# HasnainRaz/Fast-SRGAN

Hardware: AMD Instinct MI355X
Metric: SR train-step images/sec (96->384 4x, full GAN step: G+D+VGG perceptual loss) (higher is better)
Workload: dtype x3v; 1 GPU; BASELINE configs[2]: full GAN training step, 8 residual blocks / 64 filters, 96x96->384x384; per_gpu_batch=32, global_batch=32, parallelism=dp1, collectives=none, rccl_world_size=1, launch=hipGraph replay

## Files before the change

### fast-srgan_amd/csrc/conv_wgrad.hip

```cpp
#include "fsr_common.h"
#include "fsr_host.h"
#include <cstdlib>

constexpr int WGRAD_GROUP_MAX = 32;

#ifndef FSR_ABLW
#define FSR_ABLW 0
#endif

struct WgradKArgs {
  const void* x;
  const void* dy;
  float* ws;
  int N, IH, IW, CinPad;
  int OH, OW, CoutPad;
  int dy_ps;
  int tiles_x, tiles_y, tiles_total, tiles_per_slab, nslab;
  int nbm, nbn;
  int x3;
  int group_n;
  const void* gx[WGRAD_GROUP_MAX];
  const void* gdy[WGRAD_GROUP_MAX];
};

struct WgradGroupOut {
  float* dw[WGRAD_GROUP_MAX];
};

template <typename T, int BM, int BN, int S, int TPH>
constexpr bool wgrad_dma() {
  return sizeof(T) == 2 && BM >= 64 && BN == 64 && (S == 1 || TPH == 4);
}
template <typename T, int BM, int BN, int S, int TPH>
constexpr int wgrad_dma_dy_instr() {
  return (TPH * 16 * ((BM + 16) / (16 / (int)sizeof(T))) + 63) / 64;
}
template <typename T, int BM, int BN, int S, int TPH>
constexpr int wgrad_dma_halo_instr() {
  return (((TPH - 1) * S + 3) * (15 * S + 3) * ((BN + 16) / (16 / (int)sizeof(T))) + 63) / 64;
}
template <typename T, int BM, int BN, int S, int TPH>
constexpr size_t wgrad_dma_lds_bytes() {
  return (size_t)2 * 1024 * (wgrad_dma_dy_instr<T, BM, BN, S, TPH>() + wgrad_dma_halo_instr<T, BM, BN, S, TPH>());
}

template <typename T, int BM, int BN, int S, int TPH, bool X3W = false>
__global__ __launch_bounds__((BM >= 64 && BN == 64) ? 512 : 256) void conv_wgrad_kernel(const WgradKArgs a) {
  static_assert(!X3W || (BM == 128 && BN == 64 && sizeof(T) == 2), "the x3 form of the 128 x 64 block");
  constexpr int NW = (BM >= 64 && BN == 64) ? 8 : 4;
  static_assert(BM <= 64 || (BM == 128 && BN == 64 && sizeof(T) == 2), "128-row blocks: 16-bit, 64 input channels");
  constexpr int NTHR = NW * 64;
  constexpr int EPB = 16 / (int)sizeof(T);
  constexpr int PAD = 16;
  constexpr int PA = BM + PAD, PB = BN + PAD;
  constexpr int HH = (TPH - 1) * S + 3, HW = 15 * S + 3;
  constexpr int NPAIR = (BM / 16) * (BN / 16);
  constexpr int TPW = (NPAIR + NW - 1) / NW;
  constexpr int NBT = BN / 16;
  static_assert(TPW <= NBT, "a wave's pairs must share its co tile");
  constexpr int TPIX = TPH * 16;

  HIP_DYNAMIC_SHARED(char, smem)
  T* dyt = (T*)smem;
  T* halo = dyt + TPIX * PA;
  constexpr bool DMA = wgrad_dma<T, BM, BN, S, TPH>();

  const int tid = threadIdx.x, lane = tid & 63, wave = __builtin_amdgcn_readfirstlane(tid >> 6);
  const int l15 = lane & 15, lg = lane >> 4;
  int bid = a.group_n > 0 ? (int)blockIdx.x : xcd_remap((int)blockIdx.x, (int)gridDim.x);
  const int layer = a.group_n > 0 ? bid / a.nslab : 0;
  if (a.group_n > 0) bid -= layer * a.nslab;
  const int bn = bid % a.nbn;
  bid /= a.nbn;
  const int bm = bid % a.nbm;
  const int slab = bid / a.nbm;

  constexpr bool COPAIR = (BM >= 64 && BN == 64);
  const bool active = wave * TPW < NPAIR;
  const int co_t = COPAIR ? (wave / NBT) * TPW : (wave * TPW) / NBT;
  constexpr bool x3blk = X3W;
  const int ci_t0 = COPAIR ? (x3blk ? (wave + 2 * (wave / NBT)) % NBT : wave % NBT) : (wave * TPW) % NBT;
  const bool skip_lo = x3blk && ci_t0 >= 2;

  f32x4 acc[9][TPW];
#pragma unroll
  for (int t = 0; t < 9; ++t)
#pragma unroll
    for (int j = 0; j < TPW; ++j) acc[t][j] = (f32x4){0.f, 0.f, 0.f, 0.f};

  const void* xsel = a.x;
  const void* dysel = a.dy;
  if (a.group_n > 0) {
#pragma unroll
    for (int l = 0; l < WGRAD_GROUP_MAX; ++l)
      if (l == layer) {
        xsel = a.gx[l];
        dysel = a.gdy[l];
      }
  }
  const T* xg = (const T*)xsel;
  const T* dyg = (const T*)dysel;
  const int tile0 = slab * a.tiles_per_slab;
  const int tile1 = (tile0 + a.tiles_per_slab < a.tiles_total) ? tile0 + a.tiles_per_slab : a.tiles_total;

  constexpr int DUNITS = TPIX * (BM / EPB), HUNITS = HH * HW * (BN / EPB);
  constexpr int DPT = (DUNITS + NTHR - 1) / NTHR, HPT = (HUNITS + NTHR - 1) / NTHR;
  u32x4 dreg[DPT], hreg[HPT];
  auto stage_issue = [&](int tile) {
    const int tx = tile % a.tiles_x;
    const int ty = (tile / a.tiles_x) % a.tiles_y;
    const int img = tile / (a.tiles_x * a.tiles_y);
    const int oy0 = ty * TPH, ox0 = tx * 16;
#pragma unroll
    for (int i = 0; i < DPT; ++i) {
      const int u = tid + i * NTHR;
      u32x4 v = (u32x4){0u, 0u, 0u, 0u};
      if (DUNITS % NTHR == 0 || u < DUNITS) {
        const int unit = u % (BM / EPB), p = u / (BM / EPB);
        const int oy = oy0 + p / 16, ox = ox0 + (p & 15);
        if (oy < a.OH && ox < a.OW) {
          const int ch = bm * BM + unit * EPB;
          unsigned eoff;
          if (!a.dy_ps) {
            eoff = (unsigned)((img * a.OH + oy) * a.OW + ox) * (unsigned)a.CoutPad + (unsigned)ch;
          } else {
            const int cps = a.CoutPad >> 2;
            const int q = ch / cps, cc = ch - q * cps;
            eoff = (unsigned)((img * 2 * a.OH + 2 * oy + (q >> 1)) * (2 * a.OW) + 2 * ox + (q & 1)) * (unsigned)cps + (unsigned)cc;
          }
          v = *(const u32x4*)(dyg + eoff);
        }
      }
      dreg[i] = v;
    }
    const int iy0 = oy0 * S - 1, ix0 = ox0 * S - 1;
#pragma unroll
    for (int i = 0; i < HPT; ++i) {
      const int u = tid + i * NTHR;
      u32x4 v = (u32x4){0u, 0u, 0u, 0u};
      if (HUNITS % NTHR == 0 || u < HUNITS) {
        const int unit = u % (BN / EPB), p = u / (BN / EPB);
        const int iy = iy0 + p / HW, ix = ix0 + p % HW;
        if (iy >= 0 && iy < a.IH && ix >= 0 && ix < a.IW)
          v = *(const u32x4*)(xg + (unsigned)((img * a.IH + iy) * a.IW + ix) * (unsigned)a.CinPad + (unsigned)(bn * BN + unit * EPB));
      }
      hreg[i] = v;
    }
  };
  auto stage_commit = [&]() {
#pragma unroll
    for (int i = 0; i < DPT; ++i) {
      const int u = tid + i * NTHR;
      if (DUNITS % NTHR == 0 || u < DUNITS) *(u32x4*)(dyt + (u / (BM / EPB)) * PA + (u % (BM / EPB)) * EPB) = dreg[i];
    }
#pragma unroll
    for (int i = 0; i < HPT; ++i) {
      const int u = tid + i * NTHR;
      if (HUNITS % NTHR == 0 || u < HUNITS) *(u32x4*)(halo + (u / (BN / EPB)) * PB + (u % (BN / EPB)) * EPB) = hreg[i];
    }
  };

  constexpr int UPA = PA / EPB, UPB = PB / EPB;
  constexpr int DYI = wgrad_dma_dy_instr<T, BM, BN, S, TPH>(), HAI = wgrad_dma_halo_instr<T, BM, BN, S, TPH>();
  constexpr int NPIECE = DYI + HAI, IPW = (NPIECE + NW - 1) / NW;
  constexpr unsigned IMG_BYTES = NPIECE * 1024u;
  unsigned rel[DMA ? IPW : 1], pk[DMA ? IPW : 1];
  if constexpr (DMA) {
#pragma unroll
    for (int j = 0; j < IPW; ++j) {
      const int g = j * NW + wave;
      unsigned r_ = 0, k_ = 0x80000000u;
      if (g < DYI) {
        const int slot = g * 64 + lane, p_ = slot / UPA, u_ = slot - p_ * UPA;
        const int py = p_ >> 4, px = p_ & 15;
        const int ch = bm * BM + u_ * EPB;
        if (!a.dy_ps) {
          r_ = (unsigned)((py * a.OW + px) * a.CoutPad + ch);
        } else {
          const int cps = a.CoutPad >> 2;
          const int q = ch / cps, cc = ch - q * cps;
          r_ = (unsigned)(((2 * py + (q >> 1)) * (2 * a.OW) + 2 * px + (q & 1)) * cps + cc);
        }
        k_ = (unsigned)py | ((unsigned)px << 8) | ((u_ >= BM / EPB || p_ >= TPIX) ? 0x80000000u : 0u);
      } else if (g < NPIECE) {
        const int slot = (g - DYI) * 64 + lane, p_ = slot / UPB, u_ = slot - p_ * UPB;
        const int py = p_ / HW, px = p_ - py * HW;
        r_ = (unsigned)((py * a.IW + px) * a.CinPad + bn * BN + u_ * EPB);
        k_ = (unsigned)py | ((unsigned)px << 8) | ((u_ >= BN / EPB || p_ >= HH * HW) ? 0x80000000u : 0u);
      }
      rel[j] = r_;
      pk[j] = k_;
    }
  }
  const fsr_buf_t dy_buf = fsr_make_buf(dyg, DMA ? (unsigned)((size_t)a.N * a.OH * a.OW * a.CoutPad * sizeof(T)) : 0u);
  const fsr_buf_t x_buf = fsr_make_buf(xg, DMA ? (unsigned)((size_t)a.N * a.IH * a.IW * a.CinPad * sizeof(T)) : 0u);
  const fsr_lds_addr_t lds0 = FSR_LDS_ADDR(smem);
  struct DmaTile {
    int oy0, ox0, iy0, ix0;
    unsigned dy_base, x_base;
    fsr_lds_addr_t lds;
    bool on;
  };
  auto dma_tile = [&](int tile, int image, bool on) {
    DmaTile d;
    const int tx = tile % a.tiles_x;
    const int ty = (tile / a.tiles_x) % a.tiles_y;
    const int img = tile / (a.tiles_x * a.tiles_y);
    d.oy0 = ty * TPH;
    d.ox0 = tx * 16;
    d.dy_base = !a.dy_ps ? (unsigned)((img * a.OH + d.oy0) * a.OW + d.ox0) * (unsigned)a.CoutPad
                         : (unsigned)((img * 2 * a.OH + 2 * d.oy0) * (2 * a.OW) + 2 * d.ox0) * (unsigned)(a.CoutPad >> 2);
    d.iy0 = d.oy0 * S - 1;
    d.ix0 = d.ox0 * S - 1;
    d.x_base = (unsigned)((img * a.IH + d.iy0) * a.IW + d.ix0) * (unsigned)a.CinPad;
    d.lds = lds0 + (fsr_lds_addr_t)(image * IMG_BYTES);
    d.on = on;
    return d;
  };
  auto dma_piece = [&](const DmaTile& d, int j) {
    const int g = j * NW + wave;
    if (!d.on || (NPIECE % NW != 0 && g >= NPIECE)) return;
    const int py = (int)(pk[j] & 0xffu), px = (int)((pk[j] >> 8) & 0xffu);
#if FSR_ABLW == 7
    const bool keep = false;
// ... 10 lines not shown
      FSR_BLDS16(x_buf, voff, 0u, d.lds + (fsr_lds_addr_t)(g * 1024));
    }
  };
  auto dma_issue = [&](int tile, int image) {
    const DmaTile d = dma_tile(tile, image, true);
#pragma unroll
    for (int j = 0; j < IPW; ++j) dma_piece(d, j);
  };

  int image = 0;
  if constexpr (DMA) {
    if (tile0 < tile1) dma_issue(tile0, 0);
  } else {
    if (tile0 < tile1) stage_issue(tile0);
  }
  for (int tile = tile0; tile < tile1; ++tile) {
    if constexpr (DMA) {
#if FSR_ABLW != 4 && FSR_ABLW != 6
      FSR_WAIT_VM(0);
#endif
#if FSR_ABLW != 5 && FSR_ABLW != 6
      FSR_BARRIER();
#endif
#if FSR_ABLW != 1
      if (tile + 1 < tile1) dma_issue(tile + 1, image ^ 1);
#endif
      dyt = (T*)(smem + image * IMG_BYTES);
      halo = (T*)(smem + image * IMG_BYTES + DYI * 1024);
      image ^= 1;
    } else {
      __syncthreads();
#if FSR_ABLW == 1
      if (tile == tile0) stage_commit();
      __syncthreads();
#else
      stage_commit();
      __syncthreads();
      if (tile + 1 < tile1) stage_issue(tile + 1);
#endif
    }
    if (!active) continue;
#if FSR_ABLW == 2
    continue;
#endif

    if constexpr (sizeof(T) == 2 && COPAIR) {
      constexpr int NS = TPH / 2, NSTAGE = NS * 9;
      const int qrow = l15 >> 2, qch = (l15 & 3) * 4, c0 = 8 * (lg & 1);
      const T* pa_base = dyt + ((lg >> 1) * 16 + c0 + qrow) * PA + co_t * 16 + qch;
      const T* pb_base = halo + ((lg >> 1) * S * HW + (c0 + qrow) * S) * PB + ci_t0 * 16 + qch;
      auto frag = [&](const T* p0, int second) {
        const s16x4 lo = __builtin_amdgcn_ds_read_tr16_b64_v4i16(FSR_LDS_PTR(s16x4, p0));
        const s16x4 hi = __builtin_amdgcn_ds_read_tr16_b64_v4i16(FSR_LDS_PTR(s16x4, p0 + second));
        return (s16x8){lo[0], lo[1], lo[2], lo[3], hi[0], hi[1], hi[2], hi[3]};
      };
      auto xfrag = [&](int i) {
        const int ks = i / 9, t = i % 9;
        return frag(pb_base + ((ks * 2 * S + t / 3) * HW + t % 3) * PB, 4 * S * PB);
      };
      constexpr int NWH = (BM == 128) ? 2 : TPW;
      s16x8 af[2][TPW], bf[3];
#pragma unroll
      for (int w = 0; w < TPW; ++w) af[0][w] = frag(pa_base + w * 16, 4 * PA);
      bf[0] = xfrag(0);
      bf[1] = xfrag(1);
#pragma unroll
      for (int i = 0; i < NSTAGE; ++i) {
        const int ks = i / 9, t = i % 9;
        if (i + 2 < NSTAGE) bf[(i + 2) % 3] = xfrag(i + 2);
        if (t == 4 && ks + 1 < NS) {
#pragma unroll
          for (int w = 0; w < NWH; ++w) af[(ks + 1) & 1][w] = frag(pa_base + (ks + 1) * 32 * PA + w * 16, 4 * PA);
          if (!skip_lo) {
#pragma unroll
            for (int w = NWH; w < TPW; ++w) af[(ks + 1) & 1][w] = frag(pa_base + (ks + 1) * 32 * PA + w * 16, 4 * PA);
          }
        }
#pragma unroll
        for (int w = 0; w < NWH; ++w) acc[t][w] = mfma16<T>(af[ks & 1][w], bf[i % 3], acc[t][w]);
        if (!skip_lo) {
#pragma unroll
          for (int w = NWH; w < TPW; ++w) acc[t][w] = mfma16<T>(af[ks & 1][w], bf[i % 3], acc[t][w]);
        }
        __builtin_amdgcn_sched_barrier(0);
      }
    } else if constexpr (sizeof(T) == 2) {
      const int qrow = l15 >> 2, qch = (l15 & 3) * 4;
#pragma unroll 1
      for (int s = 0; s < TPH / 2; ++s) {
        const int r = 2 * s + (lg >> 1);
        const int c0 = 8 * (lg & 1);
        constexpr int NA = COPAIR ? TPW : 1;
        s16x8 af[NA];
#pragma unroll
        for (int w = 0; w < NA; ++w) {
          const T* pa = dyt + (r * 16 + c0 + qrow) * PA + (co_t + w) * 16 + qch;
          const s16x4 lo = __builtin_amdgcn_ds_read_tr16_b64_v4i16(FSR_LDS_PTR(s16x4, pa));
          const s16x4 hi = __builtin_amdgcn_ds_read_tr16_b64_v4i16(FSR_LDS_PTR(s16x4, pa + 4 * PA));
          af[w] = (s16x8){lo[0], lo[1], lo[2], lo[3], hi[0], hi[1], hi[2], hi[3]};
        }
#pragma unroll
        for (int t = 0; t < 9; ++t) {
          const int ky = t / 3, kx = t % 3;
          const T* pb0 = halo + ((r * S + ky) * HW + (c0 + qrow) * S + kx) * PB + ci_t0 * 16 + qch;
          if constexpr (COPAIR) {
#if FSR_ABLW == 3
            const s16x8 bf = af[(t + 1) & 1];
#else
            const s16x4 lo = __builtin_amdgcn_ds_read_tr16_b64_v4i16(FSR_LDS_PTR(s16x4, pb0));
            const s16x4 hi = __builtin_amdgcn_ds_read_tr16_b64_v4i16(FSR_LDS_PTR(s16x4, pb0 + 4 * S * PB));
            const s16x8 bf = (s16x8){lo[0], lo[1], lo[2], lo[3], hi[0], hi[1], hi[2], hi[3]};
#endif
#pragma unroll
            for (int w = 0; w < TPW; ++w) acc[t][w] = mfma16<T>(af[w], bf, acc[t][w]);
          } else {
#pragma unroll
            for (int j = 0; j < TPW; ++j) {
              const s16x4 lo = __builtin_amdgcn_ds_read_tr16_b64_v4i16(FSR_LDS_PTR(s16x4, pb0 + j * 16));
              const s16x4 hi = __builtin_amdgcn_ds_read_tr16_b64_v4i16(FSR_LDS_PTR(s16x4, pb0 + j * 16 + 4 * S * PB));
              const s16x8 bf = (s16x8){lo[0], lo[1], lo[2], lo[3], hi[0], hi[1], hi[2], hi[3]};
              acc[t][j] = mfma16<T>(af[0], bf, acc[t][j]);
            }
          }
        }
      }
    } else {
#pragma unroll 1
      for (int s = 0; s < TPH * 4; ++s) {
        const int r = s >> 2, c = 4 * (s & 3) + lg;
        const float av = dyt[(r * 16 + c) * PA + co_t * 16 + l15];
        const float av1 = COPAIR ? dyt[(r * 16 + c) * PA + (co_t + 1) * 16 + l15] : 0.f;
#pragma unroll
        for (int t = 0; t < 9; ++t) {
          const int ky = t / 3, kx = t % 3;
          const T* pb = halo + ((r * S + ky) * HW + c * S + kx) * PB + ci_t0 * 16 + l15;
          if constexpr (COPAIR) {
            const float bv = pb[0];
            acc[t][0] = mfma_f32_16x16x4(av, bv, acc[t][0]);
            acc[t][1] = mfma_f32_16x16x4(av1, bv, acc[t][1]);
          } else {
#pragma unroll
            for (int j = 0; j < TPW; ++j) acc[t][j] = mfma_f32_16x16x4(av, pb[j * 16], acc[t][j]);
          }
        }
      }
    }
  }

  if (!active) return;
#pragma unroll
  for (int t = 0; t < 9; ++t)
#pragma unroll
    for (int j = 0; j < TPW; ++j) {
      const int cot = COPAIR ? co_t + j : co_t, cit = COPAIR ? ci_t0 : ci_t0 + j;
      float* o = a.ws + (((size_t)(layer * a.nslab + slab) * 9 + t) * a.CoutPad + bm * BM + cot * 16 + lg * 4) * a.CinPad + bn * BN + cit * 16 + l15;
#pragma unroll
      for (int r = 0; r < 4; ++r) o[(size_t)r * a.CinPad] = acc[t][j][r];
    }
}

__global__ __launch_bounds__(256) void conv_wgrad_reduce_kernel(const float* __restrict__ ws, float* __restrict__ dw, int nslab,
                                                                int cout, int cin, int cout_pad, int cin_pad, int ps) {
  __shared__ float red[8][32];
  const int total = 9 * cout * cin;
  const size_t sstride = (size_t)9 * cout_pad * cin_pad;
  const int oi = threadIdx.x & 31, pl = threadIdx.x >> 5;
  for (int i0 = blockIdx.x * 32; i0 < total; i0 += gridDim.x * 32) {
    const int i = i0 + oi;
    float s = 0.f;
    int co = 0, ci = 0, t = 0;
    if (i < total) {
      ci = i % cin;
      co = (i / cin) % cout;
      t = i / (cin * cout);
      const int row = ps ? (co & 3) * (cout_pad >> 2) + (co >> 2) : co;
      const float* p = ws + ((size_t)t * cout_pad + row) * cin_pad + ci;
      int k = pl;
      for (; k + 24 < nslab; k += 32) {
        const float v0 = p[(size_t)k * sstride], v1 = p[(size_t)(k + 8) * sstride];
        const float v2 = p[(size_t)(k + 16) * sstride], v3 = p[(size_t)(k + 24) * sstride];
        s = ((s + v0) + v1) + v2 + v3;
      }
      for (; k < nslab; k += 8) s += p[(size_t)k * sstride];
    }
    red[pl][oi] = s;
    __syncthreads();
    if (pl == 0 && i < total) {
      float r = red[0][oi];
#pragma unroll
      for (int j = 1; j < 8; ++j) r += red[j][oi];
      dw[((size_t)co * cin + ci) * 9 + t] += r;
    }
    __syncthreads();
  }
}

__global__ __launch_bounds__(256) void conv_wgrad_reduce_x3_kernel(const float* __restrict__ ws, float* __restrict__ dw, int nslab,
                                                                   int cout, int cin, int cout_pad, int cin_pad, int ps) {
  __shared__ float red[8][32];
  const int total = 9 * cout * cin;
  const size_t sstride = (size_t)9 * cout_pad * cin_pad;
  const int oi = threadIdx.x & 31, pl = threadIdx.x >> 5;
  for (int i0 = blockIdx.x * 32; i0 < total; i0 += gridDim.x * 32) {
    const int i = i0 + oi;
    float s = 0.f;
    int co = 0, ci = 0, t = 0;
    if (i < total) {
      ci = i % cin;
      co = (i / cin) % cout;
      t = i / (cin * cout);
      const int row = ps ? (co & 3) * (cout_pad >> 3) + (co >> 2) : co;
      const int rh = (row >> 5) * 64 + (row & 31), ch = (ci >> 5) * 64 + (ci & 31);
      const float* p = ws + ((size_t)t * cout_pad + rh) * cin_pad + ch;
      const size_t rlo = (size_t)32 * cin_pad;
      float hh = 0.f, hl = 0.f, lh = 0.f;
      for (int k = pl; k < nslab; k += 8) {
        const float* q = p + (size_t)k * sstride;
        hh += q[0];
        hl += q[32];
        lh += q[rlo];
      }
      s = hh + (hl + lh);
    }
    red[pl][oi] = s;
    __syncthreads();
    if (pl == 0 && i < total) {
      float r = red[0][oi];
#pragma unroll
      for (int j = 1; j < 8; ++j) r += red[j][oi];
      dw[((size_t)co * cin + ci) * 9 + t] += r;
    }
    __syncthreads();
  }
}

namespace {

inline fsr_wgrad_desc physical_desc(const fsr_wgrad_desc* d) {
  fsr_wgrad_desc q = *d;
  if (d->dtype == FSR_X3) {
    q.dtype = FSR_BF16;
    q.cin_pad = 2 * d->cin_pad;
    q.cout_pad = 2 * d->cout_pad;
    q.cin = q.cin_pad;
    q.cout = q.cout_pad;
  }
  return q;
}

struct WgradPlan {
  int BM, BN, TPH, S;
  int tiles_x, tiles_y, tiles_total, tiles_per_slab, nslab, nbm, nbn;
  size_t lds;
};

int make_plan(const fsr_wgrad_desc* d_in, WgradPlan& p) {
  if (!d_in) return fsr_fail(-1, "conv3x3_wgrad: null descriptor");
  if (d_in->dtype == FSR_X3 && (d_in->cin_pad % 32 || d_in->cout_pad % 32 || d_in->cin > d_in->cin_pad || d_in->cout > d_in->cout_pad ||
                                (d_in->dy_pixel_shuffled && (d_in->cout_pad / 4) % 32)))
    return fsr_fail(-2, "conv3x3_wgrad: x3 tensors have a multiple of 32 channels");
  const fsr_wgrad_desc dphys = physical_desc(d_in);
  const fsr_wgrad_desc* d = &dphys;
  if (d->dtype != FSR_F32 && d->dtype != FSR_BF16 && d->dtype != FSR_F16) return fsr_fail(-2, "conv3x3_wgrad: unknown dtype %d", d->dtype);
  const int cpad = d->dtype != FSR_F32 ? 32 : 16;
  if (d->stride != 1 && d->stride != 2) return fsr_fail(-2, "conv3x3_wgrad: stride must be 1 or 2");
  if (d->cin_pad % cpad || d->cin_pad <= 0) return fsr_fail(-2, "conv3x3_wgrad: cin_pad %d is not a multiple of %d", d->cin_pad, cpad);
  if (d->cout_pad % 16 || d->cout_pad <= 0) return fsr_fail(-2, "conv3x3_wgrad: cout_pad %d is not a multiple of 16", d->cout_pad);
  if (d->dtype != FSR_F32 && d->cout_pad % 8) return fsr_fail(-2, "conv3x3_wgrad: bad cout_pad");
  if (d->cin > d->cin_pad || d->cout > d->cout_pad || d->cin <= 0 || d->cout <= 0) return fsr_fail(-2, "conv3x3_wgrad: bad channel counts");
  if (d->oh != (d->ih - 1) / d->stride + 1 || d->ow != (d->iw - 1) / d->stride + 1)
    return fsr_fail(-2, "conv3x3_wgrad: output dims do not match k=3,p=1,stride=%d", d->stride);
  if (d->dy_pixel_shuffled && (d->cout_pad % 64 || d->cout != d->cout_pad))
    return fsr_fail(-2, "conv3x3_wgrad: pixel-shuffled dy needs cout %% 64 == 0");
  if ((long long)d->n * d->ih * d->iw * d->cin_pad >= (1LL << 31) || (long long)d->n * d->oh * d->ow * d->cout_pad >= (1LL << 31))
    return fsr_fail(-2, "conv3x3_wgrad: tensors with 2^31 or more elements are not supported");
  p.S = d->stride;
  p.BM = (d->cout_pad % 64 == 0) ? 64 : 16;
  p.BN = (d->cin_pad % 64 == 0) ? 64 : (d->cin_pad % 32 == 0 ? 32 : 16);
  const char* ebm = getenv("FSR_WGRAD_BM");
  const bool bm64 = ebm && atoi(ebm) == 64;
  if (d->dtype != FSR_F32 && p.BN == 64 && d->cout_pad % 128 == 0 && !bm64) p.BM = 128;
  if (d->dy_pixel_shuffled && (d->cout_pad / 4) % (p.BM == 128 ? 64 : p.BM)) p.BM = 16;
  p.TPH = d->dtype != FSR_F32 ? 8 : 4;
  {
    const char* e2 = getenv("FSR_WGRAD_S2");
    if (d->dtype != FSR_F32 && p.S == 2 && p.BM >= 64 && p.BN == 64 && !(e2 && atoi(e2) == 8)) p.TPH = 4;
    if (p.S == 2 && p.TPH == 8 && p.BM == 128) p.BM = 64;
  }
  p.tiles_x = (d->ow + 15) / 16;
  p.tiles_y = (d->oh + p.TPH - 1) / p.TPH;
  p.tiles_total = p.tiles_x * p.tiles_y * d->n;
  p.nbm = d->cout_pad / p.BM;
  p.nbn = d->cin_pad / p.BN;
  const int target = (p.BM == 16 || p.BN < 64) ? 1024 : 256;
  int want = (target + p.nbm * p.nbn - 1) / (p.nbm * p.nbn);
  if (const char* e = getenv("FSR_WGRAD_SLABS")) {
    const int v = atoi(e);
    if (v > 0) want = v;
  }
  if (want > p.tiles_total) want = p.tiles_total;
  if (want < 1) want = 1;
  p.tiles_per_slab = (p.tiles_total + want - 1) / want;
  p.nslab = (p.tiles_total + p.tiles_per_slab - 1) / p.tiles_per_slab;
  const int es = d->dtype != FSR_F32 ? 2 : 4;
  const int HH = (p.TPH - 1) * p.S + 3, HW = 15 * p.S + 3;
  p.lds = ((size_t)p.TPH * 16 * (p.BM + 16) + (size_t)HH * HW * (p.BN + 16)) * es;
  return 0;
}

template <typename T, int BM, int BN, int S, int TPH, bool X3W = false>
int launch_wgrad(const WgradKArgs& a, size_t lds, hipStream_t stream) {
  auto kern = conv_wgrad_kernel<T, BM, BN, S, TPH, X3W>;
  static bool attr_set = false;
  if (!attr_set) {
    (void)hipFuncSetAttribute((const void*)kern, hipFuncAttributeMaxDynamicSharedMemorySize, 160 * 1024);
    attr_set = true;
  }
  if constexpr (wgrad_dma<T, BM, BN, S, TPH>()) lds = wgrad_dma_lds_bytes<T, BM, BN, S, TPH>();
  hipLaunchKernelGGL(kern, dim3((unsigned)(a.nslab * a.nbm * a.nbn * (a.group_n > 0 ? a.group_n : 1))), dim3((BM >= 64 && BN == 64) ? 512 : 256), lds, stream, a);
  return fsr_check_launch("conv_wgrad_kernel");
}

template <typename T, int TPH>
int dispatch_wgrad(const WgradPlan& p, const WgradKArgs& a, hipStream_t stream) {
  if constexpr (sizeof(T) == 2 && TPH == 8) {
    if (p.TPH == 4) {
      if (p.S != 2 || p.BN != 64) return fsr_fail(-2, "conv3x3_wgrad: 4-row tiles are a stride-2 configuration");
      if constexpr (std::is_same<T, bf16_t>::value) {
        if (p.BM == 128 && a.x3) return launch_wgrad<T, 128, 64, 2, 4, true>(a, p.lds, stream);
      }
      if (p.BM == 128) return launch_wgrad<T, 128, 64, 2, 4>(a, p.lds, stream);
      if (p.BM == 64) return launch_wgrad<T, 64, 64, 2, 4>(a, p.lds, stream);
      return fsr_fail(-2, "conv3x3_wgrad: no 4-row kernel for block %dx%d", p.BM, p.BN);
    }
  }
#define FSR_WG_CASE(bm, bn)                                                           \
  if (p.BM == bm && p.BN == bn)                                                       \
    return p.S == 1 ? launch_wgrad<T, bm, bn, 1, TPH>(a, p.lds, stream) : launch_wgrad<T, bm, bn, 2, TPH>(a, p.lds, stream);
  if constexpr (std::is_same<T, bf16_t>::value) {
    if (p.BM == 128 && p.BN == 64 && p.S == 1 && a.x3) return launch_wgrad<T, 128, 64, 1, TPH, true>(a, p.lds, stream);
  }
  if constexpr (sizeof(T) == 2) {
    if (p.BM == 128 && p.BN == 64 && p.S == 1) return launch_wgrad<T, 128, 64, 1, TPH>(a, p.lds, stream);
  }
  FSR_WG_CASE(64, 64)
  FSR_WG_CASE(64, 32)
  FSR_WG_CASE(16, 64)
  FSR_WG_CASE(16, 32)
  if constexpr (sizeof(T) == 4) {
    FSR_WG_CASE(64, 16)
    FSR_WG_CASE(16, 16)
  }
#undef FSR_WG_CASE
  return fsr_fail(-2, "conv3x3_wgrad: no kernel for block %dx%d", p.BM, p.BN);
}

}

__global__ __launch_bounds__(256) void conv_wgrad_reduce_grouped_kernel(const float* __restrict__ ws, const WgradGroupOut out, int nslab,
                                                                        int cout, int cin, int cout_pad, int cin_pad) {
  __shared__ float red[8][32];
  const int total = 9 * cout * cin;
  const size_t sstride = (size_t)9 * cout_pad * cin_pad;
  const int oi = threadIdx.x & 31, pl = threadIdx.x >> 5;
  const float* wl = ws + (size_t)blockIdx.y * nslab * sstride;
  float* dw = out.dw[0];
#pragma unroll
  for (int l = 1; l < WGRAD_GROUP_MAX; ++l)
    if (l == (int)blockIdx.y) dw = out.dw[l];
  for (int i0 = blockIdx.x * 32; i0 < total; i0 += gridDim.x * 32) {
    const int i = i0 + oi;
    float s = 0.f;
    int co = 0, ci = 0, t = 0;
    if (i < total) {
      ci = i % cin;
      co = (i / cin) % cout;
      t = i / (cin * cout);
      const float* p = wl + ((size_t)t * cout_pad + co) * cin_pad + ci;
      for (int k = pl; k < nslab; k += 8) s += p[(size_t)k * sstride];
    }
    red[pl][oi] = s;
    __syncthreads();
    if (pl == 0 && i < total) {
      float r = red[0][oi];
#pragma unroll
      for (int j = 1; j < 8; ++j) r += red[j][oi];
      dw[((size_t)co * cin + ci) * 9 + t] += r;
    }
    __syncthreads();
  }
}

static int group_slabs(const WgradPlan& p, int nlayers) {
  int wpl = 256 / nlayers;
  if (wpl < 1) wpl = 1;
  if (wpl > p.tiles_total) wpl = p.tiles_total;
  return wpl;
}

extern "C" size_t fsr_conv3x3_wgrad_grouped_workspace(const fsr_wgrad_desc* d, int nlayers) {
  WgradPlan p;
  if (nlayers < 1 || nlayers > WGRAD_GROUP_MAX || make_plan(d, p) != 0) return 0;
  return (size_t)nlayers * group_slabs(p, nlayers) * 9 * d->cout_pad * d->cin_pad * sizeof(float);
}

extern "C" int fsr_conv3x3_wgrad_grouped(const fsr_wgrad_desc* d, int nlayers, const void* const* x, const void* const* dy,
                                         float* const* dw_oihw, void* workspace, fsr_stream_t stream_) {
  hipStream_t stream = (hipStream_t)stream_;
  WgradPlan p;
  if (int rc = make_plan(d, p)) return rc;
  if (nlayers < 1 || nlayers > WGRAD_GROUP_MAX) return fsr_fail(-2, "fsr_conv3x3_wgrad_grouped: 1..%d layers per launch", WGRAD_GROUP_MAX);
  if (!x || !dy || !dw_oihw || !workspace) return fsr_fail(-1, "fsr_conv3x3_wgrad_grouped: null argument");
  if (d->dtype == FSR_X3) return fsr_fail(-2, "fsr_conv3x3_wgrad_grouped: not available for x3 tensors (launch the layers one by one)");
  if (p.nbm * p.nbn != 1 || d->dy_pixel_shuffled || d->cout != d->cout_pad || d->cin != d->cin_pad)
    return fsr_fail(-2, "fsr_conv3x3_wgrad_grouped: layers of one 64 x 64 block (cout = cin = 64, unpadded, no pixel shuffle)");
  WgradKArgs a = {};
  WgradGroupOut out = {};
  for (int l = 0; l < nlayers; ++l) {
    if (!x[l] || !dy[l] || !dw_oihw[l]) return fsr_fail(-1, "fsr_conv3x3_wgrad_grouped: null pointer for layer %d", l);
    a.gx[l] = x[l];
    a.gdy[l] = dy[l];
    out.dw[l] = dw_oihw[l];
  }
  a.group_n = nlayers;
  a.ws = (float*)workspace;
  a.N = d->n; a.IH = d->ih; a.IW = d->iw; a.CinPad = d->cin_pad;
  a.OH = d->oh; a.OW = d->ow; a.CoutPad = d->cout_pad;
  a.dy_ps = 0;
  a.tiles_x = p.tiles_x; a.tiles_y = p.tiles_y; a.tiles_total = p.tiles_total;
  a.nslab = group_slabs(p, nlayers);
  a.tiles_per_slab = (p.tiles_total + a.nslab - 1) / a.nslab;
  a.nslab = (p.tiles_total + a.tiles_per_slab - 1) / a.tiles_per_slab;
  a.nbm = a.nbn = 1;
  const int rc = d->dtype == FSR_BF16 ? dispatch_wgrad<bf16_t, 8>(p, a, stream)
                 : (d->dtype == FSR_F16 ? dispatch_wgrad<f16_t, 8>(p, a, stream) : dispatch_wgrad<float, 4>(p, a, stream));
  if (rc) return rc;
  const int total = 9 * d->cout * d->cin;
  int blocks = (total + 31) / 32;
  if (blocks > 2048) blocks = 2048;
  hipLaunchKernelGGL(conv_wgrad_reduce_grouped_kernel, dim3(blocks, nlayers), dim3(256), 0, stream, (const float*)workspace, out, a.nslab,
                     d->cout, d->cin, d->cout_pad, d->cin_pad);
  return fsr_check_launch("conv_wgrad_reduce_grouped_kernel");
}

extern "C" size_t fsr_conv3x3_wgrad_workspace(const fsr_wgrad_desc* d) {
  WgradPlan p;
  if (make_plan(d, p) != 0) return 0;
  const int f = d->dtype == FSR_X3 ? 4 : 1;
  return (size_t)p.nslab * 9 * d->cout_pad * d->cin_pad * f * sizeof(float);
}

extern "C" int fsr_conv3x3_wgrad(const fsr_wgrad_desc* d_in, const void* x, const void* dy, float* dw_oihw, void* workspace,
                                 fsr_stream_t stream_) {
  hipStream_t stream = (hipStream_t)stream_;
  WgradPlan p;
  if (int rc = make_plan(d_in, p)) return rc;
  if (!x || !dy || !dw_oihw || !workspace) return fsr_fail(-1, "fsr_conv3x3_wgrad: null argument");
  const bool x3 = d_in->dtype == FSR_X3;
  if (x3 && ((((size_t)x | (size_t)dy) & 127) != 0)) return fsr_fail(-2, "fsr_conv3x3_wgrad: x3 tensors must be 128-byte aligned");
  const fsr_wgrad_desc dphys = physical_desc(d_in);
  const fsr_wgrad_desc* d = &dphys;
  WgradKArgs a = {};
  a.x = x;
  a.dy = dy;
  a.ws = (float*)workspace;
  a.N = d->n;
  a.IH = d->ih;
  a.IW = d->iw;
  a.CinPad = d->cin_pad;
  a.OH = d->oh;
  a.OW = d->ow;
  a.CoutPad = d->cout_pad;
  a.dy_ps = d->dy_pixel_shuffled;
  a.tiles_x = p.tiles_x;
  a.tiles_y = p.tiles_y;
  a.tiles_total = p.tiles_total;
  a.tiles_per_slab = p.tiles_per_slab;
  a.nslab = p.nslab;
  a.nbm = p.nbm;
  a.nbn = p.nbn;
  a.x3 = x3 ? 1 : 0;
  int rc = d->dtype == FSR_BF16 ? dispatch_wgrad<bf16_t, 8>(p, a, stream)
           : (d->dtype == FSR_F16 ? dispatch_wgrad<f16_t, 8>(p, a, stream) : dispatch_wgrad<float, 4>(p, a, stream));
  if (rc) return rc;
  const int total = 9 * d->cout * d->cin;
  int blocks = (total + 31) / 32;
  if (blocks > 8192) blocks = 8192;
  if (x3) {
    const int total3 = 9 * d_in->cout * d_in->cin;
    int blocks3 = (total3 + 31) / 32;
    if (blocks3 > 8192) blocks3 = 8192;
    hipLaunchKernelGGL(conv_wgrad_reduce_x3_kernel, dim3(blocks3), dim3(256), 0, stream, (const float*)workspace, dw_oihw,
                       p.nslab, d_in->cout, d_in->cin, d->cout_pad, d->cin_pad, d->dy_pixel_shuffled);
    return fsr_check_launch("conv_wgrad_reduce_x3_kernel");
  }
  hipLaunchKernelGGL(conv_wgrad_reduce_kernel, dim3(blocks), dim3(256), 0, stream, (const float*)workspace, dw_oihw,
                     p.nslab, d->cout, d->cin, d->cout_pad, d->cin_pad, d->dy_pixel_shuffled);
  return fsr_check_launch("conv_wgrad_reduce_kernel");
}
```

### fast-srgan_amd/ops.py

```python
import ctypes
import math
import os
import weakref

import numpy as np
import torch

from . import _lib as L

_DT = {"f32": (L.FSR_F32, torch.float32, 16), "bf16": (L.FSR_BF16, torch.bfloat16, 32), "f16": (L.FSR_F16, torch.float16, 32),
       "x3": (L.FSR_X3, torch.float32, 32)}


class Compute:

    def __init__(self, name="f16"):
        if name not in _DT:
            raise ValueError("compute dtype must be 'bf16', 'f16', 'x3' or 'f32', got %r" % (name,))
        self.name = name
        self.code, self.torch_dtype, self.cpad = _DT[name]
        self.x3 = name == "x3"
        self.pack_dtype = torch.bfloat16 if self.x3 else self.torch_dtype
        self.pack_kmul = 2 if self.x3 else 1
        self.is16 = name in ("bf16", "f16")
# ... 127 lines not shown
    w = weight.detach()
    if w.dtype != torch.float32 or not w.is_contiguous():
        w = w.float().contiguous()
    _check_dev(w)
    if mode == PACK_C3T:
        numel = ((cin + 15) // 16 * 16) * 32
    elif mode == PACK_C3:
        numel = ((cout + 15) // 16 * 16) * 32
    else:
        numel = 9 * (rows if lin else rows_pad) * k_pad * cd.pack_kmul
    out = hit[1] if (hit is not None and hit[1].device == w.device) else None
    if out is None:
        out = torch.empty(numel, dtype=torch.float32 if (cd.x3 and mode in (PACK_C3, PACK_C3T)) else cd.pack_dtype, device=w.device)
    if lin:
        if k_pad != (cin if fwd else cout) or mode in (PACK_C3, PACK_C3T):
            raise L.FsrError("the stage-contiguous filter pack has no padding")
        L.check(L.lib().fsr_pack_conv3x3_lin(cd.code, mode, _p(w), cout, cin, lin, _p(out), _stream()), "fsr_pack_conv3x3_lin")
    elif mode == PACK_C3:
        L.check(L.lib().fsr_pack_conv3x3_c3(cd.code, _p(w), cout, _p(out), 0, _stream()), "fsr_pack_conv3x3_c3")
    elif mode == PACK_C3T:
        L.check(L.lib().fsr_pack_conv3x3_c3(cd.code, _p(w), cin, _p(out), 1, _stream()), "fsr_pack_conv3x3_c3")
    else:
        L.check(L.lib().fsr_pack_conv3x3(cd.code, mode, _p(w), cout, cin, k_pad, _p(out), _stream()), "fsr_pack_conv3x3")
    slot[1][key] = (ver, out)
    return out


_ws = {}
_const = {}


class ZeroPool:

    def __init__(self, device, nfloats=4 << 20):
        self.buf = torch.zeros(nfloats, dtype=torch.float32, device=device)
        self.off = 0
        self.active = False

    def reset(self):
        if self.off:
            self.buf[:self.off].zero_()
        self.off = 0

    def take(self, shape):
        n = 1
        for d in shape:
            n *= d
        n4 = (n + 3) // 4 * 4
        if self.off + n4 > self.buf.numel():
            return None
        t = self.buf[self.off:self.off + n].view(shape)
        self.off += n4
        return t


_zero_pool = {}


def zero_pool_reset(device):
    key = str(device)
    pool = _zero_pool.get(key)
    if pool is None:
        pool = _zero_pool[key] = ZeroPool(device)
    pool.reset()
    pool.active = True


def zero_pool_end(device):
    pool = _zero_pool.get(str(device))
    if pool is not None:
        pool.active = False


def _zeros(shape, device):
    pool = _zero_pool.get(str(device))
    if pool is not None and pool.active:
        t = pool.take(tuple(shape))
        if t is not None:
            return t
    return torch.zeros(shape, dtype=torch.float32, device=device)


def _assigned(shape, device):
    pool = _zero_pool.get(str(device))
    if pool is not None and pool.active:
        t = pool.take(tuple(shape))
        if t is not None:
            return t
    return torch.empty(shape, dtype=torch.float32, device=device)


def _const_vec(values, device):
    key = (tuple(values), str(device))
    t = _const.get(key)
    if t is None:
        t = torch.tensor(values, dtype=torch.float32, device=device)
        _const[key] = t
    return t

USE_LIN_PACK = os.environ.get("FSR_PACK_LIN", "1") != "0"
USE_SIGN_BITS = os.environ.get("FSR_SIGN_BITS", "1") != "0" and os.environ.get("FSR_S2D3", "1") != "0"
_pack_block_memo = {}
_DISPATCH_ENV = ("FSR_PERSIST_CUS", "FSR_T3_ROWS", "FSR_S2D3", "FSR_T3N_G3", "FSR_CONV_STAGE", "FSR_CONV64_S2FWD",
                 "FSR_PACK_LIN")
USE_POOL_ARGMAX = os.environ.get("FSR_POOL_ARGMAX", "1") != "0"
USE_C3_KERNELS = True

PROFILE_CONV = None


def _last_kernel():
    name = L.lib().fsr_last_kernel()
    return name.decode() if name else "?"


_ws_retired = []
_capture_seen = {}


def _workspace(nbytes, device):
    key = (str(device), _stream())
    buf = _ws.get(key)
    if buf is None or buf.numel() * 4 < nbytes:
        if buf is not None:
            if _capture_seen.get(key):
                _ws_retired.append(buf)
            old = buf.numel() * 4
            nbytes = max(nbytes, 2 * old if old < (64 << 20) else old + old // 4)
        buf = torch.empty((max(nbytes, 1 << 20) + 3) // 4, dtype=torch.float32, device=device)
        _ws[key] = buf
        _capture_seen[key] = False
    if device.type == "cuda" and torch.cuda.is_current_stream_capturing():
        _capture_seen[key] = True
    return buf


_wgrad_state = {"stream": None, "active": False, "refs": [], "group": False, "pending": {}}
USE_WGRAD_STREAM = os.environ.get("FSR_WGRAD_STREAM", "1") != "0"
USE_WGRAD_GROUP = os.environ.get("FSR_WGRAD_GROUP", "1") != "0"
WGRAD_GROUP_MAX = 32


def wgrad_stream_begin(device):
    _wgrad_state["group"] = USE_WGRAD_GROUP
    if not USE_WGRAD_STREAM or L.is_emulation() or not torch.cuda.is_available():
        return
    if _wgrad_state["stream"] is None:
        _wgrad_state["stream"] = torch.cuda.Stream(device=device)
    _wgrad_state["active"] = True


def _wgrad_defer(cd, xin, dz, cout, cin, cfg, arena):
    st = _wgrad_state
    if not st["group"] or cfg.stride != 1 or cfg.pixel_shuffle or cd.x3:
        return False
    if not (cout == cin == 64 and xin.shape[3] == 64 and dz.shape[3] == 64):
        return False
    st["pending"].setdefault((cd.code, tuple(xin.shape), str(xin.device)), []).append((cd, xin, dz, arena))
    return True


def _wgrad_flush():
    st = _wgrad_state
    pending, st["pending"] = st["pending"], {}
    lib = L.lib()
    for (_code, shape, _dev), items in pending.items():
        for i0 in range(0, len(items), WGRAD_GROUP_MAX):
            grp = items[i0:i0 + WGRAD_GROUP_MAX]
            cd, x0, dz0, _ = grp[0]
            if len(grp) == 1:
                with _on_wgrad_stream(x0, dz0):
                    conv3x3_wgrad_raw(cd, x0, dz0, 64, 64, 1, out=grp[0][3])
                continue
            n, ih, iw, _c = shape
            d = L.WgradDesc(cd.code, n, ih, iw, 64, 64, ih, iw, 64, 64, 1, 0)
            need = lib.fsr_conv3x3_wgrad_grouped_workspace(ctypes.byref(d), len(grp))
            if need == 0:
                L.check(-2, "fsr_conv3x3_wgrad_grouped_workspace")
            arr = ctypes.c_void_p * len(grp)
            xs, dys, dws = arr(*[_p(g[1]) for g in grp]), arr(*[_p(g[2]) for g in grp]), arr(*[_p(g[3]) for g in grp])
            with _on_wgrad_stream(*[t for g in grp for t in (g[1], g[2])]):
                prof = PROFILE_CONV
                if prof is not None:
                    ev0, ev1 = torch.cuda.Event(enable_timing=True), torch.cuda.Event(enable_timing=True)
                    ev0.record()
                L.check(lib.fsr_conv3x3_wgrad_grouped(ctypes.byref(d), len(grp), xs, dys, dws, _p(_workspace(need, x0.device)),
                                                      _stream()), "fsr_conv3x3_wgrad_grouped")
                if prof is not None:
                    ev1.record()
                    nbytes = len(grp) * (2 * x0.numel() * x0.element_size() + 64 * 64 * 9 * 4)
                    prof.append((ev0, ev1, len(grp) * 2.0 * n * ih * iw * 64 * 64 * 9, nbytes, "conv_wgrad_kernel", "wgrad"))


def wgrad_stream_join():
    st = _wgrad_state
    if st["pending"]:
        _wgrad_flush()
    if st["active"] and st["refs"]:
        torch.cuda.current_stream().wait_stream(st["stream"])
    st["refs"] = []


def wgrad_stream_end():
    _wgrad_state["pending"] = {}
    wgrad_stream_join()
    _wgrad_state["active"] = False
    _wgrad_state["group"] = False


class _on_wgrad_stream:

    def __init__(self, *tensors):
        self.tensors = tensors
        self.ctx = None

    def __enter__(self):
        st = _wgrad_state
        if st["active"] and self.tensors[0].is_cuda:
            st["stream"].wait_stream(torch.cuda.current_stream())
            st["refs"].append(self.tensors)
            self.ctx = torch.cuda.stream(st["stream"])
            self.ctx.__enter__()
        return self

    def __exit__(self, *exc):
        if self.ctx is not None:
            self.ctx.__exit__(*exc)
        return False


def conv3x3_raw(cd, x, wpk, cout, *, mode=L.CONV_FWD, out_hw=None, stride=1, bias=None, act=L.ACT_NONE, slope=0.0,
                prelu=None, oscale=None, pixel_shuffle=False, in_pixel_shuffled=False, out_f32=False, want_stats=False,
                want_preact=False, alg_k=None, dact_mask=None, dact_slope=0.0, out_u8=False, pool2=False, dact_add=False, dact_bits=False,
                out_i420=None):
    _check_dev(x)
    if cd.x3:
        x, dact_mask = _aligned(x), (_aligned(dact_mask) if (dact_mask is not None and not dact_bits) else dact_mask)
    n = x.shape[0]
    if in_pixel_shuffled:
        ih, iw, cin = x.shape[1] // 2, x.shape[2] // 2, x.shape[3] * 4
    else:
        ih, iw, cin = x.shape[1], x.shape[2], x.shape[3]
    if mode == L.CONV_FWD:
        oh, ow = (ih - 1) // stride + 1, (iw - 1) // stride + 1
    else:
        oh, ow = out_hw
    odt = torch.uint8 if (out_u8 or out_i420) else (torch.float32 if out_f32 else cd.torch_dtype)
    oshape = (n, 2 * oh, 2 * ow, cout // 4) if pixel_shuffle else ((n, oh // 2, ow // 2, cout) if pool2 else (n, oh, ow, cout))
    if out_i420:
        oshape = (n, oh * ow * 3 // 2)
    out = _empty(oshape, odt, x.device)
    pre = _empty(oshape, odt, x.device) if want_preact else None
    stats = _assigned((n, cout, 2), x.device) if want_stats else None
    okind = (L.OUT_NV12 if len(out_i420) > 2 and out_i420[2] else L.OUT_I420) if out_i420 else (L.OUT_U8 if out_u8 else int(out_f32))
    yuv = out_i420 or (0, 0)
    d = L.ConvDesc(cd.code, mode, n, ih, iw, cin, oh, ow, cout, stride, act, float(slope), int(pixel_shuffle),
                   int(in_pixel_shuffled), okind, int(pool2), 2 if dact_bits else int(bool(dact_add)), 0, int(yuv[0]), int(yuv[1]))
    if isinstance(wpk, FilterSpec):
        opt = ((L.OPT_BIAS if bias is not None else 0) | (L.OPT_PRELU if prelu is not None else 0) | (L.OPT_OSCALE if oscale is not None else 0)
               | (L.OPT_MASK if dact_mask is not None else 0) | (L.OPT_PREACT if want_preact else 0) | (L.OPT_STATS if want_stats else 0))
        blk = 0
        if USE_LIN_PACK:
            key = (tuple(getattr(d, f) for f, _ in d._fields_), opt, L.is_emulation(), str(x.device), L.LIB_PATH,
                   tuple(os.environ.get(v) for v in _DISPATCH_ENV))
            blk = _pack_block_memo.get(key)
            if blk is None:
                blk = L.lib().fsr_conv3x3_pack_block(ctypes.byref(d), opt)
                if blk < 0:
                    L.check(blk, "fsr_conv3x3_pack_block")
                _pack_block_memo[key] = blk
        d.pack_lin = blk
        wpk = packed_filter(cd, wpk.weight, wpk.mode, wpk.k_pad, lin=blk)
    scratch = _workspace(L.lib().fsr_conv3x3_scratch(ctypes.byref(d)), x.device) if want_stats else None
    prof = PROFILE_CONV
    if prof is not None:
        ev0, ev1 = torch.cuda.Event(enable_timing=True), torch.cuda.Event(enable_timing=True)
        ev0.record()
    L.check(L.lib().fsr_conv3x3(ctypes.byref(d), _p(x), _p(wpk), _p(bias), _p(prelu), _p(oscale), _p(dact_mask),
                                float(dact_slope), _p(out), _p(pre), _p(stats), _p(scratch), _stream()), "fsr_conv3x3")
    if prof is not None:
        ev1.record()
        k = cin if alg_k is None else alg_k
        pix = oh * ow if mode == L.CONV_FWD else ih * iw
        nbytes = x.numel() * x.element_size() + out.numel() * out.element_size() + wpk.numel() * wpk.element_size()
        if dact_mask is not None:
            nbytes += dact_mask.numel() * dact_mask.element_size()
        if pre is not None:
            nbytes += pre.numel() * pre.element_size()
        prof.append((ev0, ev1, 2.0 * n * pix * cout * k * 9, nbytes, _last_kernel(), "fwd" if mode == L.CONV_FWD else "dgrad"))
    return out, pre, stats


def conv3x3_wgrad_raw(cd, x, dy, cout, cin, stride, dy_pixel_shuffled=False, out=None):
    if cd.x3:
        x, dy = _aligned(x), _aligned(dy)
    n, ih, iw, cin_pad = x.shape
    if dy_pixel_shuffled:
        oh, ow, cout_pad = dy.shape[1] // 2, dy.shape[2] // 2, dy.shape[3] * 4
    else:
        oh, ow, cout_pad = dy.shape[1], dy.shape[2], dy.shape[3]
    d = L.WgradDesc(cd.code, n, ih, iw, cin_pad, cin, oh, ow, cout_pad, cout, stride, int(dy_pixel_shuffled))
    need = L.lib().fsr_conv3x3_wgrad_workspace(ctypes.byref(d))
    if need == 0:
        L.check(-2, "fsr_conv3x3_wgrad_workspace")
    ws = _workspace(need, x.device)
    dw = out if out is not None else torch.zeros((cout, cin, 3, 3), dtype=torch.float32, device=x.device)
    prof = PROFILE_CONV
    if prof is not None:
        ev0, ev1 = torch.cuda.Event(enable_timing=True), torch.cuda.Event(enable_timing=True)
        ev0.record()
# ... 977 lines not shown
```

Baseline: 616.6 images/s.

## Enable grouped multi-layer weight-gradient launch for x3 precision 64-channel layers

Extends the grouped wgrad path, which batches several 64->64 conv weight-gradient computations into one launch plus one reduction, to the x3 (split-bf16) dtype. It adds an x3-specific grouped reduce kernel that sums the hi/lo partial products, makes the block index remapping and slab count account for multiple M/N blocks per layer, and skips storing unused accumulator tiles. The intent is to cut per-layer launch and reduction overhead and improve occupancy for the x3 workload. In exchange it adds alignment copies via _aligned and more workspace, and reorders blocks through the XCD remap on the grouped path.

```diff
diff --git a/fast-srgan_amd/csrc/conv_wgrad.hip b/fast-srgan_amd/csrc/conv_wgrad.hip
--- a/fast-srgan_amd/csrc/conv_wgrad.hip
+++ b/fast-srgan_amd/csrc/conv_wgrad.hip
@@ -67,9 +67,10 @@
 
   const int tid = threadIdx.x, lane = tid & 63, wave = __builtin_amdgcn_readfirstlane(tid >> 6);
   const int l15 = lane & 15, lg = lane >> 4;
-  int bid = a.group_n > 0 ? (int)blockIdx.x : xcd_remap((int)blockIdx.x, (int)gridDim.x);
-  const int layer = a.group_n > 0 ? bid / a.nslab : 0;
-  if (a.group_n > 0) bid -= layer * a.nslab;
+  int bid = xcd_remap((int)blockIdx.x, (int)gridDim.x);
+  const int per_layer = a.nslab * a.nbm * a.nbn;
+  const int layer = a.group_n > 0 ? bid / per_layer : 0;
+  if (a.group_n > 0) bid -= layer * per_layer;
   const int bn = bid % a.nbn;
   bid /= a.nbn;
   const int bm = bid % a.nbm;
@@ -386,6 +387,7 @@
   for (int t = 0; t < 9; ++t)
 #pragma unroll
     for (int j = 0; j < TPW; ++j) {
+      if (X3W && j >= 2 && skip_lo) continue;
       const int cot = COPAIR ? co_t + j : co_t, cit = COPAIR ? ci_t0 : ci_t0 + j;
       float* o = a.ws + (((size_t)(layer * a.nslab + slab) * 9 + t) * a.CoutPad + bm * BM + cot * 16 + lg * 4) * a.CinPad + bn * BN + cit * 16 + l15;
 #pragma unroll
@@ -625,33 +627,88 @@
   }
 }
 
+__global__ __launch_bounds__(256) void conv_wgrad_reduce_x3_grouped_kernel(const float* __restrict__ ws, const WgradGroupOut out, int nslab,
+                                                                           int cout, int cin, int cout_pad, int cin_pad) {
+  __shared__ float red[8][32];
+  const int total = 9 * cout * cin;
+  const size_t sstride = (size_t)9 * cout_pad * cin_pad;
+  const int oi = threadIdx.x & 31, pl = threadIdx.x >> 5;
+  const float* wl = ws + (size_t)blockIdx.y * nslab * sstride;
+  float* dw = out.dw[0];
+#pragma unroll
+  for (int l = 1; l < WGRAD_GROUP_MAX; ++l)
+    if (l == (int)blockIdx.y) dw = out.dw[l];
+  for (int i0 = blockIdx.x * 32; i0 < total; i0 += gridDim.x * 32) {
+    const int i = i0 + oi;
+    float s = 0.f;
+    int co = 0, ci = 0, t = 0;
+    if (i < total) {
+      ci = i % cin;
+      co = (i / cin) % cout;
+      t = i / (cin * cout);
+      const int rh = (co >> 5) * 64 + (co & 31), ch = (ci >> 5) * 64 + (ci & 31);
+      const float* p = wl + ((size_t)t * cout_pad + rh) * cin_pad + ch;
+      const size_t rlo = (size_t)32 * cin_pad;
+      float hh = 0.f, hl = 0.f, lh = 0.f;
+      for (int k = pl; k < nslab; k += 8) {
+        const float* q = p + (size_t)k * sstride;
+        hh += q[0];
+        hl += q[32];
+        lh += q[rlo];
+      }
+      s = hh + (hl + lh);
+    }
+    red[pl][oi] = s;
+    __syncthreads();
+    if (pl == 0 && i < total) {
+      float r = red[0][oi];
+#pragma unroll
+      for (int j = 1; j < 8; ++j) r += red[j][oi];
+      dw[((size_t)co * cin + ci) * 9 + t] += r;
+    }
+    __syncthreads();
+  }
+}
+
 static int group_slabs(const WgradPlan& p, int nlayers) {
-  int wpl = 256 / nlayers;
+  int wpl = 256 / nlayers / (p.nbm * p.nbn);
   if (wpl < 1) wpl = 1;
   if (wpl > p.tiles_total) wpl = p.tiles_total;
   return wpl;
 }
 
+static bool group_x3_ok(const fsr_wgrad_desc* d, int nlayers) {
+  return nlayers >= 2 && d->cout == 64 && d->cin == 64 && d->cout_pad == 64 && d->cin_pad == 64 && d->stride == 1 && !d->dy_pixel_shuffled;
+}
+
 extern "C" size_t fsr_conv3x3_wgrad_grouped_workspace(const fsr_wgrad_desc* d, int nlayers) {
   WgradPlan p;
   if (nlayers < 1 || nlayers > WGRAD_GROUP_MAX || make_plan(d, p) != 0) return 0;
-  return (size_t)nlayers * group_slabs(p, nlayers) * 9 * d->cout_pad * d->cin_pad * sizeof(float);
-}
-
-extern "C" int fsr_conv3x3_wgrad_grouped(const fsr_wgrad_desc* d, int nlayers, const void* const* x, const void* const* dy,
+  if (d->dtype == FSR_X3 && !group_x3_ok(d, nlayers)) return 0;
+  const fsr_wgrad_desc q = physical_desc(d);
+  return (size_t)nlayers * group_slabs(p, nlayers) * 9 * q.cout_pad * q.cin_pad * sizeof(float);
+}
+
+extern "C" int fsr_conv3x3_wgrad_grouped(const fsr_wgrad_desc* d_in, int nlayers, const void* const* x, const void* const* dy,
                                          float* const* dw_oihw, void* workspace, fsr_stream_t stream_) {
   hipStream_t stream = (hipStream_t)stream_;
   WgradPlan p;
-  if (int rc = make_plan(d, p)) return rc;
+  if (int rc = make_plan(d_in, p)) return rc;
   if (nlayers < 1 || nlayers > WGRAD_GROUP_MAX) return fsr_fail(-2, "fsr_conv3x3_wgrad_grouped: 1..%d layers per launch", WGRAD_GROUP_MAX);
   if (!x || !dy || !dw_oihw || !workspace) return fsr_fail(-1, "fsr_conv3x3_wgrad_grouped: null argument");
-  if (d->dtype == FSR_X3) return fsr_fail(-2, "fsr_conv3x3_wgrad_grouped: not available for x3 tensors (launch the layers one by one)");
-  if (p.nbm * p.nbn != 1 || d->dy_pixel_shuffled || d->cout != d->cout_pad || d->cin != d->cin_pad)
+  const bool x3 = d_in->dtype == FSR_X3;
+  if (x3 && !group_x3_ok(d_in, nlayers))
+    return fsr_fail(-2, "fsr_conv3x3_wgrad_grouped: x3 takes two or more 64 -> 64 layers (unpadded, stride 1, no pixel shuffle)");
+  if ((!x3 && p.nbm * p.nbn != 1) || d_in->dy_pixel_shuffled || d_in->cout != d_in->cout_pad || d_in->cin != d_in->cin_pad)
     return fsr_fail(-2, "fsr_conv3x3_wgrad_grouped: layers of one 64 x 64 block (cout = cin = 64, unpadded, no pixel shuffle)");
+  const fsr_wgrad_desc dphys = physical_desc(d_in);
+  const fsr_wgrad_desc* d = &dphys;
   WgradKArgs a = {};
   WgradGroupOut out = {};
   for (int l = 0; l < nlayers; ++l) {
     if (!x[l] || !dy[l] || !dw_oihw[l]) return fsr_fail(-1, "fsr_conv3x3_wgrad_grouped: null pointer for layer %d", l);
+    if (x3 && ((((size_t)x[l] | (size_t)dy[l]) & 127) != 0))
+      return fsr_fail(-2, "fsr_conv3x3_wgrad_grouped: x3 tensors must be 128-byte aligned (layer %d)", l);
     a.gx[l] = x[l];
     a.gdy[l] = dy[l];
     out.dw[l] = dw_oihw[l];
@@ -665,13 +722,20 @@
   a.nslab = group_slabs(p, nlayers);
   a.tiles_per_slab = (p.tiles_total + a.nslab - 1) / a.nslab;
   a.nslab = (p.tiles_total + a.tiles_per_slab - 1) / a.tiles_per_slab;
-  a.nbm = a.nbn = 1;
+  a.nbm = p.nbm;
+  a.nbn = p.nbn;
+  a.x3 = x3 ? 1 : 0;
   const int rc = d->dtype == FSR_BF16 ? dispatch_wgrad<bf16_t, 8>(p, a, stream)
                  : (d->dtype == FSR_F16 ? dispatch_wgrad<f16_t, 8>(p, a, stream) : dispatch_wgrad<float, 4>(p, a, stream));
   if (rc) return rc;
-  const int total = 9 * d->cout * d->cin;
+  const int total = 9 * d_in->cout * d_in->cin;
   int blocks = (total + 31) / 32;
   if (blocks > 2048) blocks = 2048;
+  if (x3) {
+    hipLaunchKernelGGL(conv_wgrad_reduce_x3_grouped_kernel, dim3(blocks, nlayers), dim3(256), 0, stream, (const float*)workspace, out,
+                       a.nslab, d_in->cout, d_in->cin, d->cout_pad, d->cin_pad);
+    return fsr_check_launch("conv_wgrad_reduce_x3_grouped_kernel");
+  }
   hipLaunchKernelGGL(conv_wgrad_reduce_grouped_kernel, dim3(blocks, nlayers), dim3(256), 0, stream, (const float*)workspace, out, a.nslab,
                      d->cout, d->cin, d->cout_pad, d->cin_pad);
   return fsr_check_launch("conv_wgrad_reduce_grouped_kernel");
diff --git a/fast-srgan_amd/ops.py b/fast-srgan_amd/ops.py
--- a/fast-srgan_amd/ops.py
+++ b/fast-srgan_amd/ops.py
@@ -303,10 +303,12 @@
 
 def _wgrad_defer(cd, xin, dz, cout, cin, cfg, arena):
     st = _wgrad_state
-    if not st["group"] or cfg.stride != 1 or cfg.pixel_shuffle or cd.x3:
+    if not st["group"] or cfg.stride != 1 or cfg.pixel_shuffle:
         return False
     if not (cout == cin == 64 and xin.shape[3] == 64 and dz.shape[3] == 64):
         return False
+    if cd.x3:
+        xin, dz = _aligned(xin), _aligned(dz)
     st["pending"].setdefault((cd.code, tuple(xin.shape), str(xin.device)), []).append((cd, xin, dz, arena))
     return True
 
```

Result: no change. 621.7 images/s, median of 6 (+0.8%).
